# bioinfo-ut/GenomeTester4

Measured on AMD Instinct MI355X. Metric: k-mers merged/sec, 2-list k=25 intersection (glistcompare -i), lists resident in HBM, higher is better.
Workload: dtype u64 keys + u32 counts

## Files before the change

genometester4_amd/csrc/gt4hip_api.hip:

```cpp
#include "gt4hip_host.h"

#include <stdarg.h>
#include <stdio.h>
#include <stdlib.h>
#include <string.h>
#include <new>

using namespace gt4;

static thread_local char g_create_err[512] = "";

static void pool_flush (gt4hip_context *ctx);

int gt4hip_fail (gt4hip_context *ctx, int code, const char *fmt, ...)
{
  va_list ap;
  va_start (ap, fmt);
  vsnprintf (ctx ? ctx->err : g_create_err, 512, fmt, ap);
  va_end (ap);
  return code;
}

extern "C" const char *gt4hip_strerror (int code)
{
// ... 52 lines not shown
  ctx->n_cus = prop.multiProcessorCount;
  ctx->pool_cap = prop.totalGlobalMem / 2;
  {
    const char *e = getenv ("GT4HIP_DYNAMIC");
    ctx->dynamic = e ? atoi (e) : 0;
  }
  ctx->kway_max = 32;
  ctx->kway_enabled = 1;
  snprintf (ctx->info, sizeof ctx->info, "%s|%s|%d|%zu", prop.name, prop.gcnArchName, prop.multiProcessorCount, prop.totalGlobalMem);
  if ((e = hipStreamCreateWithFlags (&ctx->stream, hipStreamNonBlocking)) != hipSuccess) {
    delete ctx->pool;
    delete ctx;
    return gt4hip_fail (NULL, GT4HIP_ENODEVICE, "gt4hip_create: hipStreamCreate: %s", hipGetErrorString (e));
  }
  for (int i = 0; i < 4; i++) hipEventCreate (&ctx->ev[i]);
  if (hipMalloc ((void **) &ctx->ctl, sizeof (PairControl)) != hipSuccess ||
      hipHostMalloc ((void **) &ctx->ctl_host, sizeof (PairControl), hipHostMallocDefault) != hipSuccess ||
      hipMalloc ((void **) &ctx->scratch, 64) != hipSuccess ||
      hipHostMalloc ((void **) &ctx->scratch_host, 64, hipHostMallocDefault) != hipSuccess) {
    gt4hip_destroy (ctx);
    return gt4hip_fail (NULL, GT4HIP_ENOMEM, "gt4hip_create: control block allocation failed");
  }
  *out = ctx;
  return GT4HIP_OK;
}

extern "C" void gt4hip_destroy (gt4hip_context *ctx)
{
  if (!ctx) return;
  hipSetDevice (ctx->device);
  if (ctx->stream) hipStreamSynchronize (ctx->stream);
  gt4hip_io_destroy (ctx);
  gt4hip_words_free (ctx, NULL);
  gt4hip_index_free (ctx);
  gt4hip_pairs_release (ctx);
  gt4hip_locations_free (ctx);
  if (ctx->pool) {
    pool_flush (ctx);
    delete ctx->pool;
  }
  void *const dev[] = { ctx->part, ctx->kway_part, ctx->kway_cnt, ctx->kway_part2, ctx->kway_need, ctx->desc, ctx->block_sums, ctx->ctl, ctx->scratch };
  for (void *p : dev)
    if (p) hipFree (p);
  if (ctx->ctl_host) hipHostFree (ctx->ctl_host);
  if (ctx->scratch_host) hipHostFree (ctx->scratch_host);
  for (int i = 0; i < 4; i++) if (ctx->ev[i]) hipEventDestroy (ctx->ev[i]);
  if (ctx->stream) hipStreamDestroy (ctx->stream);
  delete ctx;
}

extern "C" const char *gt4hip_device_info (const gt4hip_context *ctx)
{
  return ctx ? ctx->info : "";
}

extern "C" int gt4hip_context_device (const gt4hip_context *ctx) { return ctx ? ctx->device : -1; }

extern "C" int gt4hip_trim (gt4hip_context *ctx)
{
  if (!ctx) return GT4HIP_EINVAL;
  HIPCHK (ctx, hipSetDevice (ctx->device));
// ... 17 lines not shown
{
  if (!ctx || !name) return GT4HIP_EINVAL;
  if (!strcmp (name, "two_pass")) ctx->two_pass = value != 0;
  else if (!strcmp (name, "pool")) {
    ctx->pool_enabled = value != 0 && ctx->pool;
    if (!ctx->pool_enabled) pool_flush (ctx);
  }
  else if (!strcmp (name, "pool_cap_mb")) {
    ctx->pool_cap = value > 0 ? (size_t) value << 20 : 0;
    if (ctx->pool_bytes > ctx->pool_cap) pool_flush (ctx);
  }
  else if (!strcmp (name, "grid")) ctx->grid_override = value;
  else if (!strcmp (name, "scan_group")) ctx->scan_group = (int) value;
  else if (!strcmp (name, "dynamic")) ctx->dynamic = (int) value;
  else if (!strcmp (name, "a_rows")) ctx->a_rows = (int) value;
  else if (!strcmp (name, "kway")) ctx->kway_enabled = (int) value;
  else if (!strcmp (name, "kway_max")) ctx->kway_max = value == 8 ? 8 : (value == 33 ? 33 : 32);
  else if (!strcmp (name, "kway_g")) ctx->kway_g = value;
  else if (!strcmp (name, "kway_vt")) ctx->kway_vt = value;
  else if (!strcmp (name, "spin_limit")) ctx->spin_limit = value > 0 ? (uint32_t) value : 0u;
  else if (!strcmp (name, "geom1")) ctx->force_geom = value != 0 ? 1 : 0;
  else if (!strcmp (name, "geom0")) ctx->force_geom = value != 0 ? -1 : 0;
  else return gt4hip_fail (ctx, GT4HIP_EINVAL, "unknown option %s", name);
  return GT4HIP_OK;
}

extern "C" int gt4hip_get_counter (gt4hip_context *ctx, const char *name, uint64_t *value)
{
  if (!ctx || !name || !value) return GT4HIP_EINVAL;
  if (!strcmp (name, "single_pass_fallbacks")) *value = ctx->single_pass_fallbacks;
  else if (!strcmp (name, "kway_calls")) *value = ctx->kway_calls;
  else if (!strcmp (name, "kway_overflows")) *value = ctx->kway_overflows;
  else if (!strcmp (name, "kway_declined")) *value = ctx->kway_declined;
  else if (!strcmp (name, "kway_splits")) *value = ctx->kway_splits;
  else if (!strcmp (name, "kway_shared_x100")) *value = ctx->kway_shared_x100;
  else if (!strcmp (name, "kway_width")) *value = ctx->kway_width;
  else if (!strcmp (name, "nway_kernel_us")) *value = (uint64_t) (ctx->nway_kernel_ms * 1000.0);
  else if (!strcmp (name, "nway_tiles")) *value = ctx->nway_tiles;
  else if (!strcmp (name, "nway_one_pass")) *value = (uint64_t) ctx->last_multi_one_pass;
  else if (!strcmp (name, "sort_us")) *value = (uint64_t) (ctx->sort_ms * 1000.0);
  else if (!strcmp (name, "fold_us")) *value = (uint64_t) (ctx->fold_ms * 1000.0);
  else if (!strcmp (name, "extract_us")) *value = (uint64_t) (ctx->extract_ms * 1000.0);
  else if (!strcmp (name, "maker_text_tile") || !strcmp (name, "maker_code_tile")) *value = GT4HIP_MAKER_TILE;
  else if (!strcmp (name, "table_us")) *value = (uint64_t) (ctx->table_ms * 1000.0);
  else if (!strcmp (name, "query_wide")) *value = ctx->query_wide;
// ... 316 lines not shown
```

genometester4_amd/csrc/gt4hip_device.h:

```cpp
#ifndef GT4HIP_DEVICE_H
#define GT4HIP_DEVICE_H

#include "gt4hip_internal.h"

namespace gt4 {
namespace {

constexpr int WAVE = 64;

typedef unsigned long long u64;
typedef unsigned int u32;
typedef u32 u32x4 __attribute__ ((ext_vector_type (4)));


__device__ __forceinline__ u64 load_key (const u32 *__restrict__ rec, u64 i)
{
  const u32 *p = rec + 3 * i;
  return (u64) p[0] | ((u64) p[1] << 32);
}



__device__ __forceinline__ u64 shfl_up_u64 (u64 v, int d)
{
// ... 62 lines not shown
constexpr u32 AGG_READY = 1u << 31;
constexpr u64 CARRY_READY = 1ull << 63;

__device__ __forceinline__ void publish_u32 (u32 *p, u32 v) { __hip_atomic_store (p, v, __ATOMIC_RELAXED, __HIP_MEMORY_SCOPE_AGENT); }
__device__ __forceinline__ void publish_u64 (u64 *p, u64 v) { __hip_atomic_store (p, v, __ATOMIC_RELAXED, __HIP_MEMORY_SCOPE_AGENT); }
__device__ __forceinline__ u32 peek_u32 (u32 *p) { return __hip_atomic_load (p, __ATOMIC_RELAXED, __HIP_MEMORY_SCOPE_AGENT); }
__device__ __forceinline__ u64 peek_u64 (u64 *p) { return __hip_atomic_load (p, __ATOMIC_RELAXED, __HIP_MEMORY_SCOPE_AGENT); }

#define GT4_STAMP_TID GT4_PROFILE_PHASES
#define PHASE_STAMP(i) PROF (do { __builtin_amdgcn_sched_barrier (0); u64 t_; asm volatile ("s_memtime %0\n\ts_waitcnt lgkmcnt(0)" : "=s"(t_) :: "memory"); __builtin_amdgcn_sched_barrier (0); if (tid == GT4_STAMP_TID) { ph[i] += t_ - t_last; } t_last = t_; } while (0))

constexpr u32 SPIN_LIMIT = 1u << 22;
#define GT4_SCAN_ROWS 16
constexpr int SCAN_ROWS = GT4_SCAN_ROWS;

__device__ void scanner_wave (u32 *agg, u64 *carry_out, u64 num_tiles, PairControl *ctl, int lane, u32 spin_limit)
{
  __builtin_amdgcn_s_setprio (3);
  u64 carry = 0;
  const u64 rows = (num_tiles + WAVE - 1) / WAVE;
  if (lane == 0) publish_u64 (&carry_out[0], CARRY_READY);
  u32 v[SCAN_ROWS], w[SCAN_ROWS];
  auto load_batch = [&] (u32 (&dst)[SCAN_ROWS], u64 r0) {
#pragma unroll
    for (int j = 0; j < SCAN_ROWS; j++) {
      const u64 idx = (r0 + j) * WAVE + lane;
      dst[j] = (r0 + j < rows && idx < num_tiles) ? peek_u32 (&agg[idx]) : AGG_READY;
    }
  };
  load_batch (v, 0);
  for (u64 r0 = 0; r0 < rows; r0 += SCAN_ROWS) {
    const int n = rows - r0 < (u64) SCAN_ROWS ? (int) (rows - r0) : SCAN_ROWS;
    load_batch (w, r0 + SCAN_ROWS);
    int done = 0;
    u32 spins = 0;
PROF (
    u64 st_rounds = 0, st_first = 0;
)
    for (;;) {
PROF (
      const int done_before = done;
)
#pragma unroll
      for (int j = 0; j < SCAN_ROWS; j++) {
        if (j == done && j < n && __all ((v[j] & AGG_READY) != 0)) {
          carry += dpp_wave_sum_u32 (v[j] & ~AGG_READY);
// ... 61 lines not shown
      if (++spins > spin_limit) {
        if (lane == 0) atomicOr (&ctl->error, 4u);
        return;
      }
#pragma unroll
      for (int j = 0; j < SCAN_ROWS; j++) {
        const u64 idx = (first + (i0 + j) * stride) * WAVE + lane;
        if (((pending >> j) & 1u) && !(v[j] & AGG_READY)) v[j] = peek_u32 (&agg[idx]);
      }
    }
#pragma unroll
    for (int j = 0; j < SCAN_ROWS; j++) v[j] = w[j];
  }
}

__device__ void chainer_wave (u64 *rowsum, u64 *carry_out, u64 num_tiles, PairControl *ctl, int lane, u32 spin_limit)
{
  __builtin_amdgcn_s_setprio (3);
  const u64 rows = (num_tiles + WAVE - 1) / WAVE;
  if (lane == 0) publish_u64 (&carry_out[0], CARRY_READY);
  u64 base = 0;
  u64 nv = lane < (int) (rows < (u64) WAVE ? rows : WAVE) ? peek_u64 (&rowsum[lane]) : CARRY_READY;
  for (u64 b0 = 0; b0 < rows; b0 += WAVE) {
    const u64 r = b0 + lane;
    const bool in = r < rows;
    u64 v = nv;
    {
      const u64 rn = r + WAVE;
      nv = rn < rows ? peek_u64 (&rowsum[rn]) : CARRY_READY;
    }
    int done = 0;
    u32 spins = 0;
    for (;;) {
      const u64 ready = __builtin_amdgcn_ballot_w64 ((v & CARRY_READY) != 0);
      const int lead = ~ready ? (int) __builtin_ctzll (~ready) : WAVE;
      if (lead > done) {
        const u64 inc = wave_inclusive_scan (lane < lead ? (v & ~CARRY_READY) : 0ull, lane);
        if (lane >= done && lane < lead && in) publish_u64 (&carry_out[r + 1], CARRY_READY | (base + inc));
// ... 2 lines not shown
          base += (u64) __shfl ((u32) inc, WAVE - 1, WAVE) | ((u64) __shfl ((u32) (inc >> 32), WAVE - 1, WAVE) << 32);
          break;
        }
      }
      if ((spins & 63u) == 63u && peek_u32 (&ctl->error)) spins = spin_limit;
      if (++spins > spin_limit) {
        if (lane == 0) atomicOr (&ctl->error, 4u);
        return;
      }
      if (in && !(v & CARRY_READY)) v = peek_u64 (&rowsum[r]);
    }
  }
}

__device__ __forceinline__ void scanner_part (u32 *agg, u64 *rowsum, u64 *carry_out, u64 num_tiles, PairControl *ctl, int lane, u32 spin_limit,
                                              u32 sub, u32 n_sub)
{
  if (n_sub <= 1) scanner_wave (agg, carry_out, num_tiles, ctl, lane, spin_limit);
  else if (sub == 0) chainer_wave (rowsum, carry_out, num_tiles, ctl, lane, spin_limit);
  else summer_wave (agg, rowsum, num_tiles, ctl, lane, spin_limit, sub - 1, n_sub - 1);
}

constexpr int RESOLVE_LOOKBACK = GT4_RESOLVE_LOOKBACK;

__device__ __forceinline__ u64 resolve_offset (u32 *agg, u64 *carry, u64 tile, int lane, u32 a, u64 c, PairControl *ctl, u32 spin_limit)
{
  const u64 row = tile / WAVE;
  const u32 pos = (u32) (tile % WAVE);
  u32 *const wa = &agg[row * WAVE + lane];
  u64 *const wc = &carry[row];
  const bool mine = (u32) lane < pos;
  u32 spins = 0;
PROF (
  const bool agg_ok0 = __all (!mine || (a & AGG_READY) != 0), carry_ok0 = (c & CARRY_READY) != 0;
)
// ... 91 lines not shown
```

genometester4_amd/csrc/gt4hip_host.h:

```cpp
#ifndef GT4HIP_HOST_H
#define GT4HIP_HOST_H

#include "../../include/gt4hip.h"
#include "gt4hip_internal.h"

#include <stddef.h>
#include <algorithm>
#include <utility>
#include <vector>

struct gt4hip_io;

struct gt4hip_context {
  int device;
  hipStream_t stream;
  hipEvent_t ev[4];
  int n_cus;
  int two_pass;
  int64_t grid_override;
  uint32_t spin_limit;
  int a_rows;
  int dynamic;
  int scan_group;
  int force_geom;
  uint64_t single_pass_fallbacks;
  std::vector<std::pair<void *, size_t>> *pool;
  int pool_enabled;
  size_t pool_bytes;
  size_t pool_cap;
  uint64_t *part;
  size_t part_bytes;
// ... 88 lines not shown
};

GT4HIP_LOCAL int gt4hip_output_list (gt4hip_context *ctx, int s, gt4hip_list *given, uint64_t need, uint32_t word_length, TempLists &made, gt4hip_list **out);

struct PairRun {
  uint64_t n_words[4];
  uint64_t total_count[4];
  double merge_ms, device_ms;
  uint64_t tiles;
};
GT4HIP_LOCAL int gt4hip_run_pair (gt4hip_context *ctx, const uint32_t *A, uint64_t nA, const uint32_t *B, uint64_t nB, const gt4::PairParams &p,
                                  bool count_only, uint32_t *const dst[4], PairRun *run, bool force_two_pass = false);
GT4HIP_LOCAL int gt4hip_pair_with_outputs (gt4hip_context *ctx, const gt4hip_list *a, const gt4hip_list *b, const gt4::PairParams &p, bool count_only,
                                           gt4hip_list *out[4], PairRun *run);
GT4HIP_LOCAL gt4::PairParams gt4hip_nway_params (uint32_t op_bit, uint32_t rule, uint32_t cutoff, uint32_t ovr, uint32_t filter);
GT4HIP_LOCAL size_t gt4hip_lookback_desc_bytes (uint64_t tiles);

int gt4hip_nway_union (gt4hip_context *ctx, const gt4hip_list *const lists[], uint32_t k, uint32_t rule, uint32_t cutoff, uint32_t ovr,
                       uint32_t filter, bool count_only, gt4hip_list *out, uint64_t *n_words, uint64_t *total_count, double *device_ms, int *used);
int gt4hip_nway_table (gt4hip_context *ctx, const gt4hip_list *const lists[], uint32_t k, const uint32_t cols[], gt4hip_count_table *table, int probe,
                       int presence, int *used);
int gt4hip_block_alloc (gt4hip_context *ctx, size_t bytes, void **dev, void **owner);
void gt4hip_block_free (void *owner);
int gt4hip_table_alloc (gt4hip_context *ctx, gt4hip_count_table *table, uint64_t n, uint32_t n_lists);
int gt4hip_table_set_ragged (gt4hip_context *ctx, gt4hip_count_table *table, uint64_t tiles);
void *gt4hip_table_compact_bases (gt4hip_count_table *table);
void *gt4hip_table_padded_bases (gt4hip_count_table *table);
void gt4hip_io_destroy (gt4hip_context *ctx);
#define GT4HIP_MAKER_TILE 4096u
#define GT4HIP_SUBSET_TILE 4096u
// ... 12 lines not shown
```

genometester4_amd/csrc/gt4hip_internal.h:

```cpp
#ifndef GT4HIP_INTERNAL_H
#define GT4HIP_INTERNAL_H

#include <hip/hip_runtime.h>
#include <stdint.h>

#include "gt4hip_pair_variant.h"

#ifdef GT4_PROFILE_PHASES
#define PROF(...) __VA_ARGS__
#else
#define PROF(...)
#endif

namespace gt4 {

struct PairOutputs {
  uint32_t *rec[4];
};

struct PairControl {
  unsigned long long n_words[4];
  unsigned long long total_count[4];
  unsigned int ticket;
  unsigned int error;
  unsigned int role;
  unsigned int pad;
  unsigned long long phase_cycles[24];
  unsigned long long resolve_stats[8];
};

hipError_t launch_partition (hipStream_t s, const uint32_t *A, uint64_t nA, const uint32_t *B, uint64_t nB,
                             uint64_t num_tiles, uint64_t tile_records, uint64_t *part);
hipError_t launch_pair_merge (hipStream_t s, const PairVariant &v, int grid, const uint32_t *A, uint64_t nA,
                              const uint32_t *B, uint64_t nB, const uint64_t *part, uint64_t num_tiles,
                              const PairParams &p, const PairOutputs &o, unsigned long long *desc,
                              PairControl *ctl);
hipError_t launch_scan_tiles (hipStream_t s, unsigned long long *desc, uint64_t num_tiles,
                              unsigned long long *block_sums);
hipError_t launch_generate (hipStream_t s, uint32_t *rec, uint64_t n, uint64_t stride, uint64_t seed,
                            uint64_t count_seed, uint32_t max_count, uint64_t mult, uint64_t add);
hipError_t launch_sum_counts (hipStream_t s, const uint32_t *rec, uint64_t n, unsigned long long *sum);
hipError_t launch_check_sorted (hipStream_t s, const uint32_t *rec, uint64_t n, unsigned int *bad);
hipError_t launch_lower_bound (hipStream_t s, const uint32_t *rec, uint64_t n, uint64_t key,
                               unsigned long long *idx);
hipError_t launch_extract_column (hipStream_t s, const uint32_t *rec, uint64_t n, uint32_t *counts, uint32_t n_lists, uint32_t column);
hipError_t launch_extract_keys (hipStream_t s, const uint32_t *rec, uint64_t n, unsigned long long *keys);
hipError_t launch_decode_index (hipStream_t s, const unsigned long long *kmers, uint64_t n, uint64_t num_locations, uint32_t *rec);

int merge_blocks_per_cu (const PairVariant &v);
// ... 5 lines not shown
```

genometester4_amd/csrc/gt4hip_kernels.hip:

```cpp
#define GT4_RESOLVE_LOOKBACK 3
#include "gt4hip_device.h"

#include <type_traits>

namespace gt4 {

namespace {


enum : u32 { KIND_SKIP = 0, KIND_A = 1, KIND_B = 2, KIND_BOTH = 3 };

struct StreamCoef {
  u32 m_f1, m_f2, m_min, m_max, m_sub2;
  u32 konst;
  u32 minz;
  u32 check_in;
  u32 lo;
  u32 cutoff;
  u32 subtract;
};

template <int S>
__device__ __forceinline__ StreamCoef make_coef (const PairParams &p)
{
// ... 76 lines not shown

constexpr u64 PART_COARSE = 64;

__global__ void k_partition_coarse (const u32 *__restrict__ A, u64 nA, const u32 *__restrict__ B, u64 nB, u64 num_tiles, u64 tile_records, u64 *__restrict__ coarse)
{
  const u64 c = (u64) blockIdx.x * blockDim.x + threadIdx.x;
  const u64 n_coarse = (num_tiles + PART_COARSE - 1) / PART_COARSE;
  if (c > n_coarse) return;
  const u64 total = nA + nB;
  u64 diag = c * PART_COARSE * tile_records;
  if (diag > total) diag = total;
  coarse[c] = merge_path (A, nA, B, nB, diag, 0, nA);
}

__global__ void k_partition (const u32 *__restrict__ A, u64 nA, const u32 *__restrict__ B, u64 nB,
                             u64 num_tiles, u64 tile_records, const u64 *__restrict__ coarse, u64 *__restrict__ part)
{
  const u64 t = (u64) blockIdx.x * blockDim.x + threadIdx.x;
  if (t > num_tiles) return;
  const u64 total = nA + nB;
  u64 diag = t * tile_records;
  if (diag > total) diag = total;
  const u64 c = t / PART_COARSE;
  u64 a = (t % PART_COARSE) ? merge_path (A, nA, B, nB, diag, coarse[c], coarse[c + 1]) : coarse[c], b = diag - a;
  if (a > 0 && b < nB && load_key (A, a - 1) == load_key (B, b)) b += 1;
  part[2 * t] = a;
  part[2 * t + 1] = b;
}


enum : int { STAGE_NONE = 0, STAGE_UNION = 1, STAGE_INTRSEC = 2, STAGE_ANY = 3, STAGE_UNION_LATE = 4, STAGE_COMPLEMENT = 5 };

template <int NT, int IPT, int OPS>
struct RankShared {
  static constexpr int CAP = NT * IPT;
  static constexpr int NCH = CAP / WAVE;
  static constexpr int STAGE_DW = OPS == STAGE_INTRSEC ? ((3 * (CAP / 2 + 1) + 3) & ~3)
                                  : ((OPS == STAGE_UNION || OPS == STAGE_COMPLEMENT) ? 3 * CAP
                                     : (OPS == STAGE_ANY ? 3 * (2 * CAP + 16) : (OPS == STAGE_UNION_LATE ? 3 * (CAP + 16) : 4)));
  static constexpr int STAGE_SLOTS = (OPS == STAGE_INTRSEC && IPT <= 4 && NT > 512) ? 4 : ((OPS == STAGE_ANY || OPS == STAGE_UNION_LATE) ? 1 : 2);
  alignas (16) u32 raw[3 * CAP];
  u32 stage[STAGE_SLOTS][STAGE_DW];
// ... 135 lines not shown
#pragma unroll
      for (int u = 0; u < G; u++) pv[u] = key_at (at[u] + 12u * (h - 1u));
#pragma unroll
      for (int u = 0; u < G; u++) {
        const u32 hs = h <= q4[u] ? 12u * h : 0u;
        u32 cand = at[u] + hs;
        asm volatile ("" : "+v"(cand));
        at[u] = pv[u] < ky[u] ? cand : at[u];
      }
    }
  }
#pragma unroll
  for (int u = 0; u < G; u++) lo[u] = at[u] - 4u * sbase[u];
}

struct TileRange {
  u64 a0, b0;
  u32 na, nb;
};


template <int NT, int IPT, int MODE, int OPS, int FAST = 0, int OPSET = 0>
__global__ __launch_bounds__ (NT, merge_waves_per_simd (NT, MODE, OPS, FAST)) void
k_pair_merge (const u32 *__restrict__ A, u64 nA, const u32 *__restrict__ B, u64 nB, u64 *part, u64 num_tiles,
              PairParams p, PairOutputs outs, u64 *desc, PairControl *ctl)
{
  constexpr int CAP = NT * IPT;
  constexpr int NW = NT / WAVE;
  constexpr int NCH = CAP / WAVE;
  constexpr int NLOAD4 = (3 * IPT + 3) / 4;
  constexpr bool LATE1 = OPS == 1 && IPT > 4;
  constexpr bool DEFER = OPS != 0 && !LATE1 && MODE != MODE_COUNT;
  constexpr int S0 = OPS == 2 ? 1 : (OPS == 4 ? 2 : 0);
  static_assert (OPS == 0 || OPS == 1 || OPS == 2 || OPS == 4, "specialised kernels exist for one of these outputs alone");
  constexpr bool GDEFER = (OPS == 0 || LATE1) && MODE != MODE_COUNT;
  constexpr int G = IPT % 3 == 0 ? 3 : 2;
  constexpr int F_TOP = GDEFER ? NLOAD4 + 1 : (OPS == 4 ? NLOAD4 : (OPS == 2 ? 2 : 1));
  constexpr int F_MID = (GDEFER || OPS == 4 || OPS == 2) ? 0 : 1;
  constexpr bool STAGGER = NT >= 1024;
// ... 7 lines not shown
  constexpr int KA = IPT / 2;
  constexpr bool OPAQUE_TID = A_ROWS || (OPS == 0 && !(FAST == 1 && (OPSET == 3 || OPSET == 5) && MODE != MODE_COUNT));
  int tid = threadIdx.x, lane = tid & (WAVE - 1);
  const int wid = __builtin_amdgcn_readfirstlane (tid / WAVE);
  static_assert (pair_variant_exists ({ NT, IPT, MODE, OPS, FAST, OPSET }), "not an instantiation the selection can return (a compile-time stream set belongs to the any-combination kernel)");
  const u32 ops = OPS ? (u32) OPS : (OPSET ? (u32) OPSET : p.ops);
  const bool need_b = (ops & 9u) != 0;

  const u64 n_rows = (num_tiles + WAVE - 1) / WAVE;
  const u32 spin_limit = p.spin_limit ? p.spin_limit : SPIN_LIMIT;
  u32 *const agg = reinterpret_cast<u32 *> (desc);
  u64 *const carry = desc + 2 * n_rows * WAVE;

  u32 role = 0;
  if (MODE == MODE_LOOKBACK) {
    if (tid == 0) sh.tick[0] = atomicAdd (&ctl->role, 1u);
    __syncthreads ();
    role = sh.tick[0];
    __syncthreads ();
    if (role == 0) {
      const u32 n_str = (u32) __builtin_popcount (ops);
      const u32 k = (u32) wid % n_str, sub = (u32) wid / n_str, n_sub = ((u32) NW - k + n_str - 1) / n_str;
      u32 s = 0;
      for (u32 seen = 0, b = 0; b < 4; b++)
        if ((ops >> b) & 1u) {
          if (seen == k) s = b;
          seen++;
        }
      u64 *const rowsum = carry + 4 * (n_rows + 1);
      if (sub < 8u && (p.scan_group || sub == 0))
        scanner_part (agg + (u64) s * n_rows * WAVE, rowsum + (u64) s * n_rows, carry + (u64) s * (n_rows + 1), num_tiles, ctl, lane, spin_limit, sub,
                      p.scan_group ? (n_sub > 8u ? 8u : n_sub) : 1u);
      return;
    }
  }

  u64 acc_sum0 = 0, acc_sum1 = 0, acc_sum2 = 0, acc_sum3 = 0;
  u64 blk_cnt = 0;

  const u32 n_workers = MODE == MODE_LOOKBACK ? gridDim.x - 1 : gridDim.x;
  const u32 wk = MODE == MODE_LOOKBACK ? role - 1 : blockIdx.x;
  const u32 ntl = (u32) num_tiles;
  auto tile_at = [&] (int j) -> u32 {
    const u64 t = (u64) wk + (u64) j * n_workers;
    return t < num_tiles ? (u32) t : 0xffffffffu;
  };
  auto deal = [&] (int j) -> u32 {
    if (MODE != MODE_LOOKBACK || !p.dynamic) return tile_at (j);
    const u32 t = atomicAdd (&ctl->ticket, 1u);
    return t < ntl ? t : 0xffffffffu;
  };
  u32 tk_next = 0xffffffffu;
  if (tid == 0) {
    u32 t3[3];
    for (int q = 0; q < 3; q++) t3[q] = deal (q);
    for (int q = 0; q < 2; q++) {
      sh.tile_id[q] = t3[q];
      if (t3[q] < ntl) {
        {
          const u64 e0 = part[2 * (u64) t3[q]], e1 = part[2 * (u64) t3[q] + 1], e2 = part[2 * (u64) t3[q] + 2], e3 = part[2 * (u64) t3[q] + 3];
// ... 470 lines not shown
      __syncthreads ();
      write_out_tile<NT> (outs.rec[S0], uniform64 (sh.excl[S0]), tot, sh.stage[(it + q) % LAG], tid);
    }
  }

  {
    const u64 sums[4] = { acc_sum0, acc_sum1, acc_sum2, acc_sum3 };
#pragma unroll
    for (int s = 0; s < 4; s++) {
      if (!((ops >> s) & 1u)) continue;
      const u64 v = wave_sum (sums[s]);
      if (lane == 0 && v) atomicAdd (&ctl->total_count[s], v);
      if (lane == 0 && wid == s && blk_cnt) atomicAdd (&ctl->n_words[s], blk_cnt);
    }
  }
}


constexpr int SCAN_NT = 256;
constexpr int SCAN_PER_BLOCK = SCAN_NT * 8;

__global__ __launch_bounds__ (SCAN_NT) void k_scan_reduce (const u64 *__restrict__ desc, u64 num_tiles, u64 *__restrict__ block_sums)
{
  __shared__ u64 red[4][SCAN_NT / WAVE];
  const u64 first = (u64) blockIdx.x * SCAN_PER_BLOCK;
  u64 s4[4] = { 0, 0, 0, 0 };
  for (u64 t = first + threadIdx.x; t < first + SCAN_PER_BLOCK && t < num_tiles; t += SCAN_NT)
    for (int s = 0; s < 4; s++) s4[s] += desc[4 * t + s];
  for (int s = 0; s < 4; s++) {
    const u64 v = wave_sum (s4[s]);
// ... 107 lines not shown
    rec[3 * i + 2] = (u32) (next - loc);
  }
}

inline int grid_for (u64 n, int block, int cap)
{
  u64 g = (n + block - 1) / block;
  if (g < 1) g = 1;
  if (g > (u64) cap) g = cap;
  return (int) g;
}

}


hipError_t launch_partition (hipStream_t s, const uint32_t *A, uint64_t nA, const uint32_t *B, uint64_t nB,
                             uint64_t num_tiles, uint64_t tile_records, uint64_t *part)
{
  u64 *const coarse = (u64 *) part + 2 * (num_tiles + 1);
  const u64 n_coarse = (num_tiles + PART_COARSE - 1) / PART_COARSE + 1;
  hipLaunchKernelGGL (k_partition_coarse, dim3 ((unsigned) ((n_coarse + 255) / 256)), dim3 (256), 0, s, A, nA, B, nB, num_tiles, tile_records, coarse);
  const u64 threads = num_tiles + 1;
  hipLaunchKernelGGL (k_partition, dim3 ((unsigned) ((threads + 255) / 256)), dim3 (256), 0, s, A, nA, B, nB, num_tiles, tile_records,
                      (const u64 *) coarse, (u64 *) part);
  return hipGetLastError ();
}

typedef void (*PairKernel) (const u32 *, u64, const u32 *, u64, u64 *, u64, PairParams, PairOutputs, u64 *, PairControl *);

template <int... Vs, class F>
static PairKernel lift (int v, F f)
{
  PairKernel k = nullptr;
  ((v == Vs ? (void) (k = f (std::integral_constant<int, Vs>{})) : (void) 0), ...);
  return k;
}

static PairKernel pair_kernel (const PairVariant &v)
{
  return lift<512, 1024> (v.nt, [&] (auto nt) {
    return lift<MODE_COUNT, MODE_LOOKBACK, MODE_OFFSETS> (v.mode, [&] (auto mode) {
      return lift<0, 1, 2, 4> (v.cls, [&] (auto cls) {
        return lift<0, 1, 2, 3> (v.fast, [&] (auto fast) {
// ... 16 lines not shown
  const PairKernel k = pair_kernel (v);
  if (!k) return 1;
  int &c = cache[v.nt == 1024][v.mode][v.cls][v.fast][v.opset];
  if (!c) {
    int n = 0;
    const hipError_t e = hipOccupancyMaxActiveBlocksPerMultiprocessor (&n, k, v.nt, 0);
    if (e != hipSuccess || n < 1) n = 1;
    const int by_regs = merge_waves_per_simd (v.nt, v.mode, v.cls, v.fast) * 4 / (v.nt / 64);
    if (by_regs >= 1 && n > by_regs) n = by_regs;
    c = n;
  }
  return c;
}

hipError_t launch_pair_merge (hipStream_t s, const PairVariant &v, int grid, const uint32_t *A, uint64_t nA,
                              const uint32_t *B, uint64_t nB, const uint64_t *part, uint64_t num_tiles,
                              const PairParams &p, const PairOutputs &o, unsigned long long *desc,
                              PairControl *ctl)
{
  const PairKernel k = pair_kernel (v);
  if (!k) return hipErrorInvalidDeviceFunction;
  hipLaunchKernelGGL (k, dim3 (grid), dim3 (v.nt), 0, s, A, nA, B, nB, (u64 *) part, num_tiles, p, o, desc, ctl);
  return hipGetLastError ();
}

hipError_t launch_scan_tiles (hipStream_t s, unsigned long long *desc, uint64_t num_tiles, unsigned long long *block_sums)
{
  const u64 n_blocks = (num_tiles + SCAN_PER_BLOCK - 1) / SCAN_PER_BLOCK;
  if (!n_blocks) return hipSuccess;
  hipLaunchKernelGGL (k_scan_reduce, dim3 ((unsigned) n_blocks), dim3 (SCAN_NT), 0, s, desc, num_tiles, block_sums);
  hipLaunchKernelGGL (k_scan_blocks, dim3 (1), dim3 (64), 0, s, block_sums, n_blocks);
  hipLaunchKernelGGL (k_scan_apply, dim3 ((unsigned) n_blocks), dim3 (SCAN_NT), 0, s, desc, num_tiles, block_sums);
  return hipGetLastError ();
}

hipError_t launch_generate (hipStream_t s, uint32_t *rec, uint64_t n, uint64_t stride, uint64_t seed, uint64_t count_seed,
                            uint32_t max_count, uint64_t mult, uint64_t add)
// ... 43 lines not shown
```

genometester4_amd/csrc/gt4hip_pair.hip:

```cpp
#include "gt4hip_host.h"

#include <stdio.h>
#include <string.h>

using namespace gt4;

size_t gt4hip_lookback_desc_bytes (uint64_t tiles)
{
  const uint64_t rows = (tiles + 63) / 64;
  return (((size_t) rows * 64 * 16 + (size_t) (rows + 1) * 32 + (size_t) rows * 32) + 255) & ~(size_t) 255;
}

static size_t desc_bytes_for (uint64_t tiles)
{
  const size_t two = ((size_t) tiles * 32 + 255) & ~(size_t) 255;
  return std::max (gt4hip_lookback_desc_bytes (tiles), two);
}

int gt4hip_run_pair (gt4hip_context *ctx, const uint32_t *A, uint64_t nA, const uint32_t *B, uint64_t nB, const PairParams &p_in,
                     bool count_only, uint32_t *const dst[4], PairRun *run, bool force_two_pass)
{
  if (p_in.ops == 8u) {
    PairParams q = p_in;
    q.ops = 4u;
    q.rule[2] = p_in.rule[3];
    q.subtract = 0;
    uint32_t *const d2[4] = { NULL, NULL, dst ? dst[3] : NULL, NULL };
    const int rc = gt4hip_run_pair (ctx, B, nB, A, nA, q, count_only, d2, run, force_two_pass);
    run->n_words[3] = run->n_words[2];
    run->total_count[3] = run->total_count[2];
    run->n_words[2] = run->total_count[2] = 0;
// ... 26 lines not shown
  const bool need_desc = !count_only;
  if (need_desc && (rc = gt4hip_grow (ctx, (void **) &ctx->desc, &ctx->desc_bytes, desc_bytes_for (tiles)))) return rc;
  if (two_pass) {
    const size_t nb = (size_t) ((tiles + 2047) / 2048) * 32;
    if ((rc = gt4hip_grow (ctx, (void **) &ctx->block_sums, &ctx->block_sums_bytes, nb))) return rc;
  }
  int grid = ctx->n_cus * merge_blocks_per_cu (v1);
  if (ctx->grid_override > 0) grid = (int) ctx->grid_override;
  if ((uint64_t) grid > tiles + 1) grid = (int) tiles + 1;
  int grid2 = ctx->n_cus * merge_blocks_per_cu (v2);
  if ((uint64_t) grid2 > tiles) grid2 = (int) tiles;

  PairOutputs outs;
  for (int s = 0; s < 4; s++) outs.rec[s] = (count_only || !dst) ? NULL : dst[s];

  hipStream_t st = ctx->stream;
  HIPCHK (ctx, hipEventRecord (ctx->ev[0], st));
  HIPCHK (ctx, hipMemsetAsync (ctx->ctl, 0, sizeof (PairControl), st));
  if (need_desc && !two_pass) HIPCHK (ctx, hipMemsetAsync (ctx->desc, 0, desc_bytes_for (tiles), st));
  HIPCHK (ctx, launch_partition (st, A, nA, B, nB, tiles, tile_records, ctx->part));
  HIPCHK (ctx, hipEventRecord (ctx->ev[1], st));
  if (count_only) {
    HIPCHK (ctx, launch_pair_merge (st, v1, grid, A, nA, B, nB, ctx->part, tiles, p, outs, NULL, ctx->ctl));
  } else if (two_pass) {
    HIPCHK (ctx, launch_pair_merge (st, v1, grid, A, nA, B, nB, ctx->part, tiles, p, outs, ctx->desc, ctx->ctl));
    HIPCHK (ctx, launch_scan_tiles (st, ctx->desc, tiles, ctx->block_sums));
    HIPCHK (ctx, hipMemsetAsync (ctx->ctl, 0, sizeof (PairControl), st));
    HIPCHK (ctx, launch_pair_merge (st, v2, grid2, A, nA, B, nB, ctx->part, tiles, p, outs, ctx->desc, ctx->ctl));
  } else {
    HIPCHK (ctx, launch_pair_merge (st, v1, grid, A, nA, B, nB, ctx->part, tiles, p, outs, ctx->desc, ctx->ctl));
  }
  HIPCHK (ctx, hipEventRecord (ctx->ev[2], st));
  HIPCHK (ctx, hipMemcpyAsync (ctx->ctl_host, ctx->ctl, sizeof (PairControl), hipMemcpyDeviceToHost, st));
  HIPCHK (ctx, hipEventRecord (ctx->ev[3], st));
  HIPCHK (ctx, hipStreamSynchronize (st));
  float ms = 0;
  if (hipEventElapsedTime (&ms, ctx->ev[1], ctx->ev[2]) == hipSuccess) run->merge_ms = ms;
  if (hipEventElapsedTime (&ms, ctx->ev[0], ctx->ev[3]) == hipSuccess) run->device_ms = ms;
PROF (
  {
    static const char *names[8] = { "p0 wait+lds", "B0", "ring+fetch issue", "p1 rank", "B1", "p2 scan/publish", "B2+out+B3+scatter", "housekeeping" };
    unsigned long long tot = 0;
    for (int i = 0; i < 8; i++) tot += ctx->ctl_host->phase_cycles[i];
    fprintf (stderr, "[phases] tiles %llu merge %.3f ms:", (unsigned long long) tiles, run->merge_ms);
    for (int i = 0; i < 8; i++) fprintf (stderr, " %s %.1f%%", names[i], tot ? 100.0 * ctx->ctl_host->phase_cycles[i] / tot : 0.0);
    fprintf (stderr, " | avg cycles/tile %.0f\n", tiles ? (double) tot / tiles : 0.0);
    const unsigned long long *rs = ctx->ctl_host->resolve_stats;
    if (rs[0]) fprintf (stderr, "[resolve] sampled %llu avg spins %.2f first-look agg-not-ready %.1f%% carry-not-ready %.1f%% | [scanner] rows %llu polling rounds %llu rows complete at batch load %llu\n", rs[0], (double) rs[1] / rs[0], 100.0 * rs[3] / rs[0], 100.0 * rs[4] / rs[0], rs[7], rs[5], rs[6]);
  }
)
  if (ctx->ctl_host->error) {
    const unsigned flags = ctx->ctl_host->error;
// ... 82 lines not shown
```

Measured before the change: 367.1 billion.

## Segment pair merge into launches overlapping partition on a side stream

Adds optional segmentation of the lookback pair merge into several launches over geometrically growing tile ranges. The partition for the next segment runs on a low-priority side stream so it overlaps the current merge, and the scanner resumes the carry chain from the segment's first row. The aim is to hide partition latency behind merge work. With default settings only one segment is used, but the kernels gain an error peek and an exit atomic per block, and partition becomes a separate strided launch.

Result: no change. 366.9 billion (-0.1%).

```diff
diff --git a/genometester4_amd/csrc/gt4hip_api.hip b/genometester4_amd/csrc/gt4hip_api.hip
--- a/genometester4_amd/csrc/gt4hip_api.hip
+++ b/genometester4_amd/csrc/gt4hip_api.hip
@@ -90,6 +90,17 @@
     return gt4hip_fail (NULL, GT4HIP_ENODEVICE, "gt4hip_create: hipStreamCreate: %s", hipGetErrorString (e));
   }
   for (int i = 0; i < 4; i++) hipEventCreate (&ctx->ev[i]);
+  {
+    int least = 0, greatest = 0;
+    if (hipDeviceGetStreamPriorityRange (&least, &greatest) != hipSuccess) least = greatest = 0;
+    bool ok = hipStreamCreateWithPriority (&ctx->side, hipStreamNonBlocking, least) == hipSuccess;
+    for (int i = 0; i < GT4HIP_PAIR_SEG_MAX; i++) ok = ok && hipEventCreateWithFlags (&ctx->ev_side[i], hipEventDisableTiming) == hipSuccess;
+    for (int i = 0; i <= GT4HIP_PAIR_SEG_MAX; i++) ok = ok && hipEventCreate (&ctx->ev_merge[i]) == hipSuccess;
+    if (!ok) {
+      gt4hip_destroy (ctx);
+      return gt4hip_fail (NULL, GT4HIP_ENODEVICE, "gt4hip_create: side stream and events: %s", hipGetErrorString (hipGetLastError ()));
+    }
+  }
   if (hipMalloc ((void **) &ctx->ctl, sizeof (PairControl)) != hipSuccess ||
       hipHostMalloc ((void **) &ctx->ctl_host, sizeof (PairControl), hipHostMallocDefault) != hipSuccess ||
       hipMalloc ((void **) &ctx->scratch, 64) != hipSuccess ||
@@ -106,6 +117,7 @@
   if (!ctx) return;
   hipSetDevice (ctx->device);
   if (ctx->stream) hipStreamSynchronize (ctx->stream);
+  if (ctx->side) hipStreamSynchronize (ctx->side);
   gt4hip_io_destroy (ctx);
   gt4hip_words_free (ctx, NULL);
   gt4hip_index_free (ctx);
@@ -121,6 +133,9 @@
   if (ctx->ctl_host) hipHostFree (ctx->ctl_host);
   if (ctx->scratch_host) hipHostFree (ctx->scratch_host);
   for (int i = 0; i < 4; i++) if (ctx->ev[i]) hipEventDestroy (ctx->ev[i]);
+  for (int i = 0; i < GT4HIP_PAIR_SEG_MAX; i++) if (ctx->ev_side[i]) hipEventDestroy (ctx->ev_side[i]);
+  for (int i = 0; i <= GT4HIP_PAIR_SEG_MAX; i++) if (ctx->ev_merge[i]) hipEventDestroy (ctx->ev_merge[i]);
+  if (ctx->side) hipStreamDestroy (ctx->side);
   if (ctx->stream) hipStreamDestroy (ctx->stream);
   delete ctx;
 }
@@ -168,6 +183,10 @@
   else if (!strcmp (name, "scan_group")) ctx->scan_group = (int) value;
   else if (!strcmp (name, "dynamic")) ctx->dynamic = (int) value;
   else if (!strcmp (name, "a_rows")) ctx->a_rows = (int) value;
+  else if (!strcmp (name, "pair_segments")) {
+    if (value < 0 || value > GT4HIP_PAIR_SEG_MAX) return gt4hip_fail (ctx, GT4HIP_EINVAL, "pair_segments: 0 .. %d", GT4HIP_PAIR_SEG_MAX);
+    ctx->pair_segments = (int) value;
+  }
   else if (!strcmp (name, "kway")) ctx->kway_enabled = (int) value;
   else if (!strcmp (name, "kway_max")) ctx->kway_max = value == 8 ? 8 : (value == 33 ? 33 : 32);
   else if (!strcmp (name, "kway_g")) ctx->kway_g = value;
@@ -183,6 +202,7 @@
 {
   if (!ctx || !name || !value) return GT4HIP_EINVAL;
   if (!strcmp (name, "single_pass_fallbacks")) *value = ctx->single_pass_fallbacks;
+  else if (!strcmp (name, "pair_merge_launches")) *value = ctx->pair_merge_launches;
   else if (!strcmp (name, "kway_calls")) *value = ctx->kway_calls;
   else if (!strcmp (name, "kway_overflows")) *value = ctx->kway_overflows;
   else if (!strcmp (name, "kway_declined")) *value = ctx->kway_declined;
diff --git a/genometester4_amd/csrc/gt4hip_device.h b/genometester4_amd/csrc/gt4hip_device.h
--- a/genometester4_amd/csrc/gt4hip_device.h
+++ b/genometester4_amd/csrc/gt4hip_device.h
@@ -100,12 +100,13 @@
 #define GT4_SCAN_ROWS 16
 constexpr int SCAN_ROWS = GT4_SCAN_ROWS;
 
-__device__ void scanner_wave (u32 *agg, u64 *carry_out, u64 num_tiles, PairControl *ctl, int lane, u32 spin_limit)
+__device__ void scanner_wave (u32 *agg, u64 *carry_out, u64 num_tiles, PairControl *ctl, int lane, u32 spin_limit, u64 first_row = 0)
 {
   __builtin_amdgcn_s_setprio (3);
   u64 carry = 0;
   const u64 rows = (num_tiles + WAVE - 1) / WAVE;
-  if (lane == 0) publish_u64 (&carry_out[0], CARRY_READY);
+  if (first_row) carry = peek_u64 (&carry_out[first_row]) & ~CARRY_READY;
+  else if (lane == 0) publish_u64 (&carry_out[0], CARRY_READY);
   u32 v[SCAN_ROWS], w[SCAN_ROWS];
   auto load_batch = [&] (u32 (&dst)[SCAN_ROWS], u64 r0) {
 #pragma unroll
@@ -114,8 +115,8 @@
       dst[j] = (r0 + j < rows && idx < num_tiles) ? peek_u32 (&agg[idx]) : AGG_READY;
     }
   };
-  load_batch (v, 0);
-  for (u64 r0 = 0; r0 < rows; r0 += SCAN_ROWS) {
+  load_batch (v, first_row);
+  for (u64 r0 = first_row; r0 < rows; r0 += SCAN_ROWS) {
     const int n = rows - r0 < (u64) SCAN_ROWS ? (int) (rows - r0) : SCAN_ROWS;
     load_batch (w, r0 + SCAN_ROWS);
     int done = 0;
@@ -207,14 +208,15 @@
   }
 }
 
-__device__ void chainer_wave (u64 *rowsum, u64 *carry_out, u64 num_tiles, PairControl *ctl, int lane, u32 spin_limit)
+__device__ void chainer_wave (u64 *rowsum, u64 *carry_out, u64 num_tiles, PairControl *ctl, int lane, u32 spin_limit, u64 first_row = 0)
 {
   __builtin_amdgcn_s_setprio (3);
   const u64 rows = (num_tiles + WAVE - 1) / WAVE;
-  if (lane == 0) publish_u64 (&carry_out[0], CARRY_READY);
   u64 base = 0;
-  u64 nv = lane < (int) (rows < (u64) WAVE ? rows : WAVE) ? peek_u64 (&rowsum[lane]) : CARRY_READY;
-  for (u64 b0 = 0; b0 < rows; b0 += WAVE) {
+  if (first_row) base = peek_u64 (&carry_out[first_row]) & ~CARRY_READY;
+  else if (lane == 0) publish_u64 (&carry_out[0], CARRY_READY);
+  u64 nv = first_row + lane < rows ? peek_u64 (&rowsum[first_row + lane]) : CARRY_READY;
+  for (u64 b0 = first_row; b0 < rows; b0 += WAVE) {
     const u64 r = b0 + lane;
     const bool in = r < rows;
     u64 v = nv;
@@ -247,11 +249,11 @@
 }
 
 __device__ __forceinline__ void scanner_part (u32 *agg, u64 *rowsum, u64 *carry_out, u64 num_tiles, PairControl *ctl, int lane, u32 spin_limit,
-                                              u32 sub, u32 n_sub)
-{
-  if (n_sub <= 1) scanner_wave (agg, carry_out, num_tiles, ctl, lane, spin_limit);
-  else if (sub == 0) chainer_wave (rowsum, carry_out, num_tiles, ctl, lane, spin_limit);
-  else summer_wave (agg, rowsum, num_tiles, ctl, lane, spin_limit, sub - 1, n_sub - 1);
+                                              u32 sub, u32 n_sub, u64 first_row = 0)
+{
+  if (n_sub <= 1) scanner_wave (agg, carry_out, num_tiles, ctl, lane, spin_limit, first_row);
+  else if (sub == 0) chainer_wave (rowsum, carry_out, num_tiles, ctl, lane, spin_limit, first_row);
+  else summer_wave (agg, rowsum, num_tiles, ctl, lane, spin_limit, (u32) first_row + sub - 1, n_sub - 1);
 }
 
 constexpr int RESOLVE_LOOKBACK = GT4_RESOLVE_LOOKBACK;
diff --git a/genometester4_amd/csrc/gt4hip_host.h b/genometester4_amd/csrc/gt4hip_host.h
--- a/genometester4_amd/csrc/gt4hip_host.h
+++ b/genometester4_amd/csrc/gt4hip_host.h
@@ -9,12 +9,18 @@
 #include <utility>
 #include <vector>
 
+#define GT4HIP_PAIR_SEG_MAX 8
+
 struct gt4hip_io;
 
 struct gt4hip_context {
   int device;
   hipStream_t stream;
   hipEvent_t ev[4];
+  hipStream_t side;
+  hipEvent_t ev_side[GT4HIP_PAIR_SEG_MAX], ev_merge[GT4HIP_PAIR_SEG_MAX + 1];
+  uint64_t pair_merge_launches;
+  int pair_segments;
   int n_cus;
   int two_pass;
   int64_t grid_override;
@@ -133,6 +139,7 @@
 GT4HIP_LOCAL int gt4hip_pair_with_outputs (gt4hip_context *ctx, const gt4hip_list *a, const gt4hip_list *b, const gt4::PairParams &p, bool count_only,
                                            gt4hip_list *out[4], PairRun *run);
 GT4HIP_LOCAL gt4::PairParams gt4hip_nway_params (uint32_t op_bit, uint32_t rule, uint32_t cutoff, uint32_t ovr, uint32_t filter);
+GT4HIP_LOCAL int gt4hip_pair_segment_cuts (int option, uint64_t tiles, uint64_t cut[GT4HIP_PAIR_SEG_MAX + 1]);
 GT4HIP_LOCAL size_t gt4hip_lookback_desc_bytes (uint64_t tiles);
 
 int gt4hip_nway_union (gt4hip_context *ctx, const gt4hip_list *const lists[], uint32_t k, uint32_t rule, uint32_t cutoff, uint32_t ovr,
diff --git a/genometester4_amd/csrc/gt4hip_internal.h b/genometester4_amd/csrc/gt4hip_internal.h
--- a/genometester4_amd/csrc/gt4hip_internal.h
+++ b/genometester4_amd/csrc/gt4hip_internal.h
@@ -24,15 +24,17 @@
   unsigned int ticket;
   unsigned int error;
   unsigned int role;
-  unsigned int pad;
+  unsigned int left;
   unsigned long long phase_cycles[24];
   unsigned long long resolve_stats[8];
 };
 
+hipError_t launch_partition_coarse (hipStream_t s, const uint32_t *A, uint64_t nA, const uint32_t *B, uint64_t nB,
+                                    uint64_t num_tiles, uint64_t tile_records, uint64_t *part);
 hipError_t launch_partition (hipStream_t s, const uint32_t *A, uint64_t nA, const uint32_t *B, uint64_t nB,
-                             uint64_t num_tiles, uint64_t tile_records, uint64_t *part);
+                             uint64_t num_tiles, uint64_t tile_begin, uint64_t tile_end, uint64_t tile_records, uint64_t *part, unsigned max_blocks = 0);
 hipError_t launch_pair_merge (hipStream_t s, const PairVariant &v, int grid, const uint32_t *A, uint64_t nA,
-                              const uint32_t *B, uint64_t nB, const uint64_t *part, uint64_t num_tiles,
+                              const uint32_t *B, uint64_t nB, const uint64_t *part, uint64_t num_tiles, uint64_t tile_begin, uint64_t tile_end,
                               const PairParams &p, const PairOutputs &o, unsigned long long *desc,
                               PairControl *ctl);
 hipError_t launch_scan_tiles (hipStream_t s, unsigned long long *desc, uint64_t num_tiles,
diff --git a/genometester4_amd/csrc/gt4hip_kernels.hip b/genometester4_amd/csrc/gt4hip_kernels.hip
--- a/genometester4_amd/csrc/gt4hip_kernels.hip
+++ b/genometester4_amd/csrc/gt4hip_kernels.hip
@@ -114,18 +114,18 @@
 }
 
 __global__ void k_partition (const u32 *__restrict__ A, u64 nA, const u32 *__restrict__ B, u64 nB,
-                             u64 num_tiles, u64 tile_records, const u64 *__restrict__ coarse, u64 *__restrict__ part)
-{
-  const u64 t = (u64) blockIdx.x * blockDim.x + threadIdx.x;
-  if (t > num_tiles) return;
+                             u64 tile_begin, u64 tile_end, u64 tile_records, const u64 *__restrict__ coarse, u64 *__restrict__ part)
+{
   const u64 total = nA + nB;
-  u64 diag = t * tile_records;
-  if (diag > total) diag = total;
-  const u64 c = t / PART_COARSE;
-  u64 a = (t % PART_COARSE) ? merge_path (A, nA, B, nB, diag, coarse[c], coarse[c + 1]) : coarse[c], b = diag - a;
-  if (a > 0 && b < nB && load_key (A, a - 1) == load_key (B, b)) b += 1;
-  part[2 * t] = a;
-  part[2 * t + 1] = b;
+  for (u64 t = tile_begin + (u64) blockIdx.x * blockDim.x + threadIdx.x; t <= tile_end; t += (u64) gridDim.x * blockDim.x) {
+    u64 diag = t * tile_records;
+    if (diag > total) diag = total;
+    const u64 c = t / PART_COARSE;
+    u64 a = (t % PART_COARSE) ? merge_path (A, nA, B, nB, diag, coarse[c], coarse[c + 1]) : coarse[c], b = diag - a;
+    if (a > 0 && b < nB && load_key (A, a - 1) == load_key (B, b)) b += 1;
+    part[2 * t] = a;
+    part[2 * t + 1] = b;
+  }
 }
 
 
@@ -291,6 +291,14 @@
   for (int u = 0; u < G; u++) lo[u] = at[u] - 4u * sbase[u];
 }
 
+__device__ __forceinline__ void leave_launch (PairControl *ctl, u32 groups, u32 tile_end)
+{
+  if (__hip_atomic_fetch_add (&ctl->left, 1u, __ATOMIC_ACQ_REL, __HIP_MEMORY_SCOPE_AGENT) != groups - 1u) return;
+  __hip_atomic_store (&ctl->ticket, tile_end, __ATOMIC_RELAXED, __HIP_MEMORY_SCOPE_AGENT);
+  __hip_atomic_store (&ctl->role, 0u, __ATOMIC_RELAXED, __HIP_MEMORY_SCOPE_AGENT);
+  __hip_atomic_store (&ctl->left, 0u, __ATOMIC_RELAXED, __HIP_MEMORY_SCOPE_AGENT);
+}
+
 struct TileRange {
   u64 a0, b0;
   u32 na, nb;
@@ -299,7 +307,7 @@
 
 template <int NT, int IPT, int MODE, int OPS, int FAST = 0, int OPSET = 0>
 __global__ __launch_bounds__ (NT, merge_waves_per_simd (NT, MODE, OPS, FAST)) void
-k_pair_merge (const u32 *__restrict__ A, u64 nA, const u32 *__restrict__ B, u64 nB, u64 *part, u64 num_tiles,
+k_pair_merge (const u32 *__restrict__ A, u64 nA, const u32 *__restrict__ B, u64 nB, u64 *part, u64 num_tiles, u32 tile_begin, u32 tile_end,
               PairParams p, PairOutputs outs, u64 *desc, PairControl *ctl)
 {
   constexpr int CAP = NT * IPT;
@@ -337,11 +345,17 @@
 
   u32 role = 0;
   if (MODE == MODE_LOOKBACK) {
-    if (tid == 0) sh.tick[0] = atomicAdd (&ctl->role, 1u);
+    if (tid == 0) {
+      sh.tick[1] = peek_u32 (&ctl->error);
+      sh.tick[0] = atomicAdd (&ctl->role, 1u);
+    }
     __syncthreads ();
     role = sh.tick[0];
+    const bool dead = sh.tick[1] != 0;
     __syncthreads ();
+    if (dead) return;
     if (role == 0) {
+      if (tid == 0) leave_launch (ctl, gridDim.x, tile_end);
       const u32 n_str = (u32) __builtin_popcount (ops);
       const u32 k = (u32) wid % n_str, sub = (u32) wid / n_str, n_sub = ((u32) NW - k + n_str - 1) / n_str;
       u32 s = 0;
@@ -352,8 +366,8 @@
         }
       u64 *const rowsum = carry + 4 * (n_rows + 1);
       if (sub < 8u && (p.scan_group || sub == 0))
-        scanner_part (agg + (u64) s * n_rows * WAVE, rowsum + (u64) s * n_rows, carry + (u64) s * (n_rows + 1), num_tiles, ctl, lane, spin_limit, sub,
-                      p.scan_group ? (n_sub > 8u ? 8u : n_sub) : 1u);
+        scanner_part (agg + (u64) s * n_rows * WAVE, rowsum + (u64) s * n_rows, carry + (u64) s * (n_rows + 1), tile_end, ctl, lane, spin_limit, sub,
+                      p.scan_group ? (n_sub > 8u ? 8u : n_sub) : 1u, tile_begin / WAVE);
       return;
     }
   }
@@ -363,10 +377,11 @@
 
   const u32 n_workers = MODE == MODE_LOOKBACK ? gridDim.x - 1 : gridDim.x;
   const u32 wk = MODE == MODE_LOOKBACK ? role - 1 : blockIdx.x;
-  const u32 ntl = (u32) num_tiles;
+  const u32 ntl = tile_end;
+  const u64 wk0 = (u64) (MODE == MODE_LOOKBACK ? tile_begin : 0u) + wk;
   auto tile_at = [&] (int j) -> u32 {
-    const u64 t = (u64) wk + (u64) j * n_workers;
-    return t < num_tiles ? (u32) t : 0xffffffffu;
+    const u64 t = wk0 + (u64) j * n_workers;
+    return t < (u64) ntl ? (u32) t : 0xffffffffu;
   };
   auto deal = [&] (int j) -> u32 {
     if (MODE != MODE_LOOKBACK || !p.dynamic) return tile_at (j);
@@ -867,6 +882,7 @@
       if (lane == 0 && wid == s && blk_cnt) atomicAdd (&ctl->n_words[s], blk_cnt);
     }
   }
+  if (MODE == MODE_LOOKBACK && tid == 0) leave_launch (ctl, gridDim.x, tile_end);
 }
 
 
@@ -1004,19 +1020,28 @@
 }
 
 
-hipError_t launch_partition (hipStream_t s, const uint32_t *A, uint64_t nA, const uint32_t *B, uint64_t nB,
-                             uint64_t num_tiles, uint64_t tile_records, uint64_t *part)
+hipError_t launch_partition_coarse (hipStream_t s, const uint32_t *A, uint64_t nA, const uint32_t *B, uint64_t nB,
+                                    uint64_t num_tiles, uint64_t tile_records, uint64_t *part)
 {
   u64 *const coarse = (u64 *) part + 2 * (num_tiles + 1);
   const u64 n_coarse = (num_tiles + PART_COARSE - 1) / PART_COARSE + 1;
   hipLaunchKernelGGL (k_partition_coarse, dim3 ((unsigned) ((n_coarse + 255) / 256)), dim3 (256), 0, s, A, nA, B, nB, num_tiles, tile_records, coarse);
-  const u64 threads = num_tiles + 1;
-  hipLaunchKernelGGL (k_partition, dim3 ((unsigned) ((threads + 255) / 256)), dim3 (256), 0, s, A, nA, B, nB, num_tiles, tile_records,
-                      (const u64 *) coarse, (u64 *) part);
   return hipGetLastError ();
 }
 
-typedef void (*PairKernel) (const u32 *, u64, const u32 *, u64, u64 *, u64, PairParams, PairOutputs, u64 *, PairControl *);
+hipError_t launch_partition (hipStream_t s, const uint32_t *A, uint64_t nA, const uint32_t *B, uint64_t nB,
+                             uint64_t num_tiles, uint64_t tile_begin, uint64_t tile_end, uint64_t tile_records, uint64_t *part, unsigned max_blocks)
+{
+  const u64 *const coarse = (const u64 *) part + 2 * (num_tiles + 1);
+  const u64 threads = tile_end - tile_begin + 1;
+  u64 blocks = (threads + 255) / 256;
+  if (max_blocks && blocks > max_blocks) blocks = max_blocks;
+  hipLaunchKernelGGL (k_partition, dim3 ((unsigned) blocks), dim3 (256), 0, s, A, nA, B, nB, tile_begin, tile_end, tile_records,
+                      coarse, (u64 *) part);
+  return hipGetLastError ();
+}
+
+typedef void (*PairKernel) (const u32 *, u64, const u32 *, u64, u64 *, u64, u32, u32, PairParams, PairOutputs, u64 *, PairControl *);
 
 template <int... Vs, class F>
 static PairKernel lift (int v, F f)
@@ -1063,13 +1088,15 @@
 }
 
 hipError_t launch_pair_merge (hipStream_t s, const PairVariant &v, int grid, const uint32_t *A, uint64_t nA,
-                              const uint32_t *B, uint64_t nB, const uint64_t *part, uint64_t num_tiles,
+                              const uint32_t *B, uint64_t nB, const uint64_t *part, uint64_t num_tiles, uint64_t tile_begin, uint64_t tile_end,
                               const PairParams &p, const PairOutputs &o, unsigned long long *desc,
                               PairControl *ctl)
 {
   const PairKernel k = pair_kernel (v);
   if (!k) return hipErrorInvalidDeviceFunction;
-  hipLaunchKernelGGL (k, dim3 (grid), dim3 (v.nt), 0, s, A, nA, B, nB, (u64 *) part, num_tiles, p, o, desc, ctl);
+  if (tile_begin > tile_end || tile_end > num_tiles || ((tile_begin || tile_end != num_tiles) && (v.mode != MODE_LOOKBACK || tile_begin % WAVE || (tile_end % WAVE && tile_end != num_tiles))))
+    return hipErrorInvalidValue;
+  hipLaunchKernelGGL (k, dim3 (grid), dim3 (v.nt), 0, s, A, nA, B, nB, (u64 *) part, num_tiles, (u32) tile_begin, (u32) tile_end, p, o, desc, ctl);
   return hipGetLastError ();
 }
 
diff --git a/genometester4_amd/csrc/gt4hip_pair.hip b/genometester4_amd/csrc/gt4hip_pair.hip
--- a/genometester4_amd/csrc/gt4hip_pair.hip
+++ b/genometester4_amd/csrc/gt4hip_pair.hip
@@ -15,6 +15,29 @@
 {
   const size_t two = ((size_t) tiles * 32 + 255) & ~(size_t) 255;
   return std::max (gt4hip_lookback_desc_bytes (tiles), two);
+}
+
+constexpr int PAIR_SEG_AUTO = 1;
+constexpr int PAIR_SIDE_BLOCKS = 2;
+
+int gt4hip_pair_segment_cuts (int option, uint64_t tiles, uint64_t cut[GT4HIP_PAIR_SEG_MAX + 1])
+{
+  int K = option > 0 ? option : PAIR_SEG_AUTO;
+  if (K > GT4HIP_PAIR_SEG_MAX) K = GT4HIP_PAIR_SEG_MAX;
+  const uint64_t rows = (tiles + 63) / 64;
+  uint64_t den = 7;
+  for (int j = 1; j < K; j++) den *= 8;
+  uint64_t pow8 = 1;
+  cut[0] = 0;
+  for (int j = 1; j < K; j++) {
+    pow8 *= 8;
+    uint64_t r = rows * (pow8 - 1) / den;
+    if (r < (uint64_t) j) r = (uint64_t) j;
+    if (r > rows) r = rows;
+    cut[j] = std::min (tiles, r * 64);
+  }
+  cut[K] = tiles;
+  return K;
 }
 
 int gt4hip_run_pair (gt4hip_context *ctx, const uint32_t *A, uint64_t nA, const uint32_t *B, uint64_t nB, const PairParams &p_in,
@@ -71,28 +94,58 @@
   PairOutputs outs;
   for (int s = 0; s < 4; s++) outs.rec[s] = (count_only || !dst) ? NULL : dst[s];
 
+  uint64_t cut[GT4HIP_PAIR_SEG_MAX + 1];
+  const int n_seg = (count_only || two_pass) ? 1 : gt4hip_pair_segment_cuts (ctx->pair_segments, tiles, cut);
   hipStream_t st = ctx->stream;
   HIPCHK (ctx, hipEventRecord (ctx->ev[0], st));
   HIPCHK (ctx, hipMemsetAsync (ctx->ctl, 0, sizeof (PairControl), st));
-  if (need_desc && !two_pass) HIPCHK (ctx, hipMemsetAsync (ctx->desc, 0, desc_bytes_for (tiles), st));
-  HIPCHK (ctx, launch_partition (st, A, nA, B, nB, tiles, tile_records, ctx->part));
-  HIPCHK (ctx, hipEventRecord (ctx->ev[1], st));
-  if (count_only) {
-    HIPCHK (ctx, launch_pair_merge (st, v1, grid, A, nA, B, nB, ctx->part, tiles, p, outs, NULL, ctx->ctl));
-  } else if (two_pass) {
-    HIPCHK (ctx, launch_pair_merge (st, v1, grid, A, nA, B, nB, ctx->part, tiles, p, outs, ctx->desc, ctx->ctl));
-    HIPCHK (ctx, launch_scan_tiles (st, ctx->desc, tiles, ctx->block_sums));
-    HIPCHK (ctx, hipMemsetAsync (ctx->ctl, 0, sizeof (PairControl), st));
-    HIPCHK (ctx, launch_pair_merge (st, v2, grid2, A, nA, B, nB, ctx->part, tiles, p, outs, ctx->desc, ctx->ctl));
+  int n_merge_ev = 0;
+  if (n_seg > 1) {
+    hipStream_t sd = ctx->side;
+    HIPCHK (ctx, hipMemsetAsync (ctx->desc, 0, desc_bytes_for (tiles), sd));
+    HIPCHK (ctx, hipEventRecord (ctx->ev_side[0], sd));
+    HIPCHK (ctx, launch_partition_coarse (st, A, nA, B, nB, tiles, tile_records, ctx->part));
+    HIPCHK (ctx, launch_partition (st, A, nA, B, nB, tiles, cut[0], cut[1], tile_records, ctx->part));
+    for (int k = 0; k < n_seg; k++) {
+      if (cut[k] == cut[k + 1]) continue;
+      HIPCHK (ctx, hipStreamWaitEvent (st, ctx->ev_side[k], 0));
+      HIPCHK (ctx, hipEventRecord (ctx->ev_merge[n_merge_ev++], st));
+      if (k + 1 < n_seg && cut[k + 1] < cut[k + 2]) {
+        HIPCHK (ctx, hipStreamWaitEvent (sd, ctx->ev_merge[n_merge_ev - 1], 0));
+        HIPCHK (ctx, launch_partition (sd, A, nA, B, nB, tiles, cut[k + 1], cut[k + 2], tile_records, ctx->part, (unsigned) (PAIR_SIDE_BLOCKS * ctx->n_cus)));
+        HIPCHK (ctx, hipEventRecord (ctx->ev_side[k + 1], sd));
+      }
+      const uint64_t seg_tiles = cut[k + 1] - cut[k];
+      const int g = (uint64_t) grid > seg_tiles + 1 ? (int) seg_tiles + 1 : grid;
+      HIPCHK (ctx, launch_pair_merge (st, v1, g, A, nA, B, nB, ctx->part, tiles, cut[k], cut[k + 1], p, outs, ctx->desc, ctx->ctl));
+    }
+    HIPCHK (ctx, hipEventRecord (ctx->ev_merge[n_merge_ev], st));
   } else {
-    HIPCHK (ctx, launch_pair_merge (st, v1, grid, A, nA, B, nB, ctx->part, tiles, p, outs, ctx->desc, ctx->ctl));
-  }
-  HIPCHK (ctx, hipEventRecord (ctx->ev[2], st));
+    if (need_desc && !two_pass) HIPCHK (ctx, hipMemsetAsync (ctx->desc, 0, desc_bytes_for (tiles), st));
+    HIPCHK (ctx, launch_partition_coarse (st, A, nA, B, nB, tiles, tile_records, ctx->part));
+    HIPCHK (ctx, launch_partition (st, A, nA, B, nB, tiles, 0, tiles, tile_records, ctx->part));
+    HIPCHK (ctx, hipEventRecord (ctx->ev[1], st));
+    if (count_only) {
+      HIPCHK (ctx, launch_pair_merge (st, v1, grid, A, nA, B, nB, ctx->part, tiles, 0, tiles, p, outs, NULL, ctx->ctl));
+    } else if (two_pass) {
+      HIPCHK (ctx, launch_pair_merge (st, v1, grid, A, nA, B, nB, ctx->part, tiles, 0, tiles, p, outs, ctx->desc, ctx->ctl));
+      HIPCHK (ctx, launch_scan_tiles (st, ctx->desc, tiles, ctx->block_sums));
+      HIPCHK (ctx, hipMemsetAsync (ctx->ctl, 0, sizeof (PairControl), st));
+      HIPCHK (ctx, launch_pair_merge (st, v2, grid2, A, nA, B, nB, ctx->part, tiles, 0, tiles, p, outs, ctx->desc, ctx->ctl));
+    } else {
+      HIPCHK (ctx, launch_pair_merge (st, v1, grid, A, nA, B, nB, ctx->part, tiles, 0, tiles, p, outs, ctx->desc, ctx->ctl));
+    }
+    HIPCHK (ctx, hipEventRecord (ctx->ev[2], st));
+  }
   HIPCHK (ctx, hipMemcpyAsync (ctx->ctl_host, ctx->ctl, sizeof (PairControl), hipMemcpyDeviceToHost, st));
   HIPCHK (ctx, hipEventRecord (ctx->ev[3], st));
   HIPCHK (ctx, hipStreamSynchronize (st));
+  if (!count_only && !two_pass) ctx->pair_merge_launches = n_seg > 1 ? (uint64_t) n_merge_ev : 1;
   float ms = 0;
-  if (hipEventElapsedTime (&ms, ctx->ev[1], ctx->ev[2]) == hipSuccess) run->merge_ms = ms;
+  if (n_seg > 1) {
+    for (int i = 0; i < n_merge_ev; i++)
+      if (hipEventElapsedTime (&ms, ctx->ev_merge[i], ctx->ev_merge[i + 1]) == hipSuccess) run->merge_ms += ms;
+  } else if (hipEventElapsedTime (&ms, ctx->ev[1], ctx->ev[2]) == hipSuccess) run->merge_ms = ms;
   if (hipEventElapsedTime (&ms, ctx->ev[0], ctx->ev[3]) == hipSuccess) run->device_ms = ms;
 PROF (
   {
```
